# tanwanirahul/surreal

Hardware: AMD Instinct MI355X
Metric: PPO learner env-steps/sec/node (GAE+update) at 1/2/4/8 GPUs; % HBM roofline (higher is better)
Workload: dtype f32; 1 GPU; C3: synthetic PPO learner batch, reference PPO defaults (LSTM 100, horizon 5, heads 300x200, n_step 25, adapt, z-filter, 10/10 epochs), SawyerLift state dims (obs 42, act 8), 1024 segments split over 1 GPU(s) (1024 per GPU); segments_per_gpu=1024, n_step=25, env_steps_per_learn_per_gpu=25600, global_segments=1024, parallelism=single, epochs_run_last=10, ppo_mode=adapt, launch=hipGraph replay

## Files before the change

surreal_amd/csrc/lstm_mfma.hip:

```cpp
#include "smi_device.hpp"
#include "smi_internal.hpp"
#include "lstm_cell.hpp"

namespace smi {

constexpr int LR = 16;
#ifdef SMI_PROF
__device__ unsigned long long g_lstm_ticks[8];
#endif

__host__ __device__ inline int lstm_ld(int k) {
  int l = round4(k);
  if ((l & 7) != 4) l += 4;
  return l;
}

__host__ __device__ inline int lstm_q(int K) { return (((K + 3) >> 2) + 3) & ~3; }

constexpr int MAXUT = 4;
__global__ void __launch_bounds__(kWG)
lstm_fwd_kernel(LstmFwdArgs a) {
  if (a.skip && a.skip[0] != 0) return;
  const int keepS = a.keep > 0 ? a.keep : a.S;
  extern __shared__ __attribute__((aligned(16))) float sm[];
  const int H = a.H, B = a.B, G4 = 4 * H;
  const int LDH = lstm_ld(4 * lstm_q(H));
  float* hA[2] = {sm, sm + LR * LDH};
  const int lane = threadIdx.x & 63, wave = threadIdx.x >> 6;
  const int li = lane & 15, lk = lane >> 4;
  const int r0 = blockIdx.x * LR;
  const int NUT = (H + 15) >> 4;
  const int64_t BH = (int64_t)B * H;
  for (int e = threadIdx.x; e < LR * LDH; e += kWG) {
    const int r = e / LDH, k = e - r * LDH;
    const bool ok = k < H && r0 + r < B;
    const float v = ok ? a.h0[(int64_t)(r0 + r) * H + k] : 0.f;
    hA[0][e] = v;
    hA[1][e] = 0.f;
    if (ok) a.hbuf[(int64_t)(r0 + r) * H + k] = v;
  }
  float creg[MAXUT][4];
#pragma unroll
  for (int u = 0; u < MAXUT; ++u) {
    const int unit = (wave + 4 * u) * 16 + li;
#pragma unroll
    for (int i = 0; i < 4; ++i) {
      const int gr = r0 + lk * 4 + i;
      const bool ok = unit < H && gr < B;
      creg[u][i] = ok ? a.c0[(int64_t)gr * H + unit] : 0.f;
      if (ok && a.cbuf) a.cbuf[(int64_t)gr * H + unit] = creg[u][i];
    }
  }
  const float* wrow[MAXUT][4];
  float bh[MAXUT][4];
#pragma unroll
  for (int u = 0; u < MAXUT; ++u) {
    int unit = (wave + 4 * u) * 16 + li;
    unit = unit < H ? unit : H - 1;
#pragma unroll
    for (int g = 0; g < 4; ++g) {
      wrow[u][g] = a.w_hh + (int64_t)(g * H + unit) * H;
      bh[u][g] = a.b_hh[g * H + unit];
    }
  }
  const int nks = (H + 3) >> 2;
  __syncthreads();
  for (int t = 0; t < a.S; ++t) {
    const float* hp = hA[t & 1];
    float* hn = hA[(t + 1) & 1];
    float xp[MAXUT][4][4];
#pragma unroll
    for (int u = 0; u < MAXUT; ++u) {
      int unit = (wave + 4 * u) * 16 + li;
      unit = unit < H ? unit : H - 1;
#pragma unroll
      for (int i = 0; i < 4; ++i) {
        int gr = r0 + lk * 4 + i;
        gr = gr < B ? gr : B - 1;
        const float* xr = a.xproj + ((int64_t)t * B + gr) * G4 + unit;
#pragma unroll
        for (int g = 0; g < 4; ++g) xp[u][g][i] = xr[g * H];
      }
    }
    f32x4 acc[MAXUT][4];
#pragma unroll
    for (int u = 0; u < MAXUT; ++u)
#pragma unroll
      for (int g = 0; g < 4; ++g) acc[u][g] = f32x4{0.f, 0.f, 0.f, 0.f};
    const float* ap = hp + li * LDH + lk;
    int ks = 0;
    for (; ks + 4 <= nks; ks += 4) {
      float av[4], bv[MAXUT][4][4];
#pragma unroll
      for (int s = 0; s < 4; ++s) {
        const int k = (ks + s) * 4 + lk;
        const int kc = k < H ? k : H - 1;
        av[s] = ap[(ks + s) * 4];
#pragma unroll
        for (int u = 0; u < MAXUT; ++u)
#pragma unroll
          for (int g = 0; g < 4; ++g) bv[u][g][s] = wrow[u][g][kc];
      }
#pragma unroll
      for (int s = 0; s < 4; ++s)
#pragma unroll
        for (int u = 0; u < MAXUT; ++u)
#pragma unroll
          for (int g = 0; g < 4; ++g) acc[u][g] = mfma4(av[s], bv[u][g][s], acc[u][g]);
    }
    for (; ks < nks; ++ks) {
      const int k = ks * 4 + lk;
      const int kc = k < H ? k : H - 1;
      const float av = ap[ks * 4];
#pragma unroll
      for (int u = 0; u < MAXUT; ++u)
#pragma unroll
        for (int g = 0; g < 4; ++g) acc[u][g] = mfma4(av, wrow[u][g][kc], acc[u][g]);
    }
#pragma unroll
    for (int u = 0; u < MAXUT; ++u) {
      const int ut = wave + 4 * u;
      const int unit = ut * 16 + li;
      if (ut >= NUT) continue;
#pragma unroll
      for (int i = 0; i < 4; ++i) {
        const int row = lk * 4 + i, gr = r0 + row;
        const float gi = xp[u][0][i] + (acc[u][0][i] + bh[u][0]);
        const float gf = xp[u][1][i] + (acc[u][1][i] + bh[u][1]);
        const float gg = xp[u][2][i] + (acc[u][2][i] + bh[u][2]);
        const float go = xp[u][3][i] + (acc[u][3][i] + bh[u][3]);
        const float ig = sigm(gi), fg = sigm(gf), cg = ftanh(gg), og = sigm(go);
        const float c = fg * creg[u][i] + ig * cg;
        const float h = og * ftanh(c);
        const bool ok = unit < H && gr < B;
        creg[u][i] = ok ? c : 0.f;
        if (unit < H) hn[row * LDH + unit] = ok ? h : 0.f;
        if (ok) {
          a.hbuf[(int64_t)(t + 1) * BH + (int64_t)gr * H + unit] = h;
          if (a.cbuf && t < keepS) a.cbuf[(int64_t)(t + 1) * BH + (int64_t)gr * H + unit] = c;
          if (a.gates && t < keepS) {
            float* gp = a.gates + ((int64_t)t * B + gr) * G4 + unit;
            gp[0] = ig; gp[H] = fg; gp[2 * H] = cg; gp[3 * H] = og;
          }
        }
      }
    }
    __syncthreads();
  }
}



__global__ void __launch_bounds__(kWG)
lstm_bwd_kernel(LstmBwdArgs a) {
  if (a.skip && a.skip[0] != 0) return;
  extern __shared__ __attribute__((aligned(16))) float sm[];
  const int H = a.H, B = a.B, G4 = 4 * H;
  const int LDG = lstm_ld(G4);
  float* dG[2] = {sm, sm + LR * LDG};
  const int lane = threadIdx.x & 63, wave = threadIdx.x >> 6;
  const int li = lane & 15, lk = lane >> 4;
  const int r0 = blockIdx.x * LR;
  const int NUT = (H + 15) >> 4;
  const int64_t BH = (int64_t)B * H;
  for (int e = threadIdx.x; e < 2 * LR * LDG; e += kWG) sm[e] = 0.f;
  float dcreg[MAXUT][4];
  f32x4 dhrec[MAXUT];
#pragma unroll
  for (int u = 0; u < MAXUT; ++u) {
    dhrec[u] = f32x4{0.f, 0.f, 0.f, 0.f};
#pragma unroll
    for (int i = 0; i < 4; ++i) dcreg[u][i] = 0.f;
  }
  int ucl[MAXUT];
#pragma unroll
  for (int u = 0; u < MAXUT; ++u) {
    const int unit = (wave + 4 * u) * 16 + li;
    ucl[u] = unit < H ? unit : H - 1;
  }
  const int nks = G4 >> 2;
  __syncthreads();
  for (int t = a.S - 1; t >= 0; --t) {
    float* dg = dG[t & 1];
#pragma unroll
    for (int u = 0; u < MAXUT; ++u) {
      const int ut = wave + 4 * u;
      const int unit = ut * 16 + li;
      if (ut >= NUT) continue;
#pragma unroll
      for (int i = 0; i < 4; ++i) {
        const int row = lk * 4 + i;
        int gr = r0 + row;
        const bool ok = unit < H && gr < B;
        gr = gr < B ? gr : B - 1;
        const int uc = ucl[u];
        const float* gp = a.gates + ((int64_t)t * B + gr) * G4 + uc;
        const float ig = gp[0], fg = gp[H], cg = gp[2 * H], og = gp[3 * H];
        const float c = a.cbuf[(int64_t)(t + 1) * BH + (int64_t)gr * H + uc];
        const float cp = a.cbuf[(int64_t)t * BH + (int64_t)gr * H + uc];
        const float dh = a.dh[(int64_t)t * BH + (int64_t)gr * H + uc] + dhrec[u][i];
        const float tc = ftanh(c);
        const float dc = dh * og * (1.f - tc * tc) + dcreg[u][i];
        const float d_o = (dh * tc) * (og * (1.f - og));
        const float d_i = (dc * cg) * (ig * (1.f - ig));
        const float d_g = (dc * ig) * (1.f - cg * cg);
        const float d_f = (dc * cp) * (fg * (1.f - fg));
        dcreg[u][i] = ok ? dc * fg : 0.f;
        if (ok) {
          float* o = a.dgates + ((int64_t)t * B + gr) * G4 + unit;
          o[0] = d_i; o[H] = d_f; o[2 * H] = d_g; o[3 * H] = d_o;
          float* l = dg + row * LDG + unit;
          l[0] = d_i; l[H] = d_f; l[2 * H] = d_g; l[3 * H] = d_o;
        }
      }
    }
    __syncthreads();
    if (t == 0) break;
#pragma unroll
    for (int u = 0; u < MAXUT; ++u) dhrec[u] = f32x4{0.f, 0.f, 0.f, 0.f};
    const float* ap = dg + li * LDG + lk;
    int ks = 0;
    for (; ks + 8 <= nks; ks += 8) {
      float av[8], bv[MAXUT][8];
#pragma unroll
      for (int s = 0; s < 8; ++s) {
        const int k = (ks + s) * 4 + lk;
        av[s] = ap[(ks + s) * 4];
#pragma unroll
        for (int u = 0; u < MAXUT; ++u) bv[u][s] = a.w_hh[(int64_t)k * H + ucl[u]];
      }
#pragma unroll
      for (int s = 0; s < 8; ++s)
#pragma unroll
        for (int u = 0; u < MAXUT; ++u) dhrec[u] = mfma4(av[s], bv[u][s], dhrec[u]);
    }
    for (; ks < nks; ++ks) {
      const int k = ks * 4 + lk;
      const float av = ap[ks * 4];
#pragma unroll
      for (int u = 0; u < MAXUT; ++u) dhrec[u] = mfma4(av, a.w_hh[(int64_t)k * H + ucl[u]], dhrec[u]);
    }
  }
}

constexpr int kWG8 = 512;
template <int N>
__device__ __forceinline__ void load_row(const float* r, int n, float* dst) {
  static_assert(N % 4 == 0, "rows in float4 runs");
  const uintptr_t ad = reinterpret_cast<uintptr_t>(r);
  if ((ad & 15) == 0 && (n & 3) == 0) {
#pragma unroll
    for (int k = 0; k < N; k += 4) {
      const float4 v = k < n ? *reinterpret_cast<const float4*>(r + k) : float4{0.f, 0.f, 0.f, 0.f};
      dst[k] = v.x; dst[k + 1] = v.y; dst[k + 2] = v.z; dst[k + 3] = v.w;
    }
  } else if ((ad & 7) == 0 && (n & 1) == 0) {
#pragma unroll
    for (int k = 0; k < N; k += 2) {
      const float2 v = k < n ? *reinterpret_cast<const float2*>(r + k) : float2{0.f, 0.f};
      dst[k] = v.x; dst[k + 1] = v.y;
    }
  } else {
#pragma unroll
    for (int k = 0; k < N; ++k) dst[k] = k < n ? r[k] : 0.f;
  }
}

constexpr int LR4 = 4;
constexpr int LSTM_HQ = 4;

__device__ __forceinline__ f32x4 mfma4x64(float a, float b, f32x4 c) {
  return __builtin_amdgcn_mfma_f32_4x4x1f32(a, b, c, 4, 0, 0);
}

__device__ __attribute__((aligned(16))) float g_lstm_zero4[4] = {0.f, 0.f, 0.f, 0.f};
template <int N, int V>
__device__ __forceinline__ void load_row_v(const float* r, int n, float* dst) {
  static_assert(N % 4 == 0 && (V == 4 || V == 2), "vector rows");
#pragma unroll
  for (int k = 0; k < N; k += V) {
    const float* src = k < n ? r + k : g_lstm_zero4;
    if constexpr (V == 4) {
      const float4 v = *reinterpret_cast<const float4*>(src);
      dst[k] = v.x; dst[k + 1] = v.y; dst[k + 2] = v.z; dst[k + 3] = v.w;
    } else {
      const float2 v = *reinterpret_cast<const float2*>(src);
      dst[k] = v.x; dst[k + 1] = v.y;
    }
  }
}

template <int N>
__device__ __forceinline__ void load_col(const float* t, int n, int ld, uint32_t zoff, int col,
                                         float* dst) {
#pragma unroll
  for (int k = 0; k < N; ++k) {
    const uint32_t row = k < n ? (uint32_t)(k * ld) : zoff;
    dst[k] = t[row + (uint32_t)col];
  }
}

template <int KP, int KX, bool VF = false, bool IMG = false>
__global__ void __launch_bounds__(kWG8)
lstm_fwd_r4_kernel(LstmFwdArgs a) {
  if (a.skip && a.skip[0] != 0) return;
  LSTM_T0();
  const int keepS = a.keep > 0 ? a.keep : a.S;
  constexpr int KXS = KX > 0 ? KX : 8;
  __shared__ __attribute__((aligned(16))) float hS[2][LR4 * KP];
  __shared__ __attribute__((aligned(16))) float xS[2][LR4 * KXS];
  __shared__ float pre[LR4][4 * KP];
  const int H = a.H, B = a.B, G4 = 4 * H;
  const int tid = threadIdx.x, lane = tid & 63, wave = tid >> 6;
  const int r0 = blockIdx.x * LR4;
  const int64_t BH = (int64_t)B * H;
  const int col = wave * 64 + lane;
  const bool cact = wave * 64 < G4;
  const int colc = col < G4 ? col : G4 - 1;
  float w[KP];
  float wx[KXS];
  float bh = a.b_hh[colc];
  if constexpr (KX > 0) bh += a.b_ih[colc];
  if constexpr (IMG) {
    load_col<KP>(a.w_hh, H, G4, (uint32_t)(H * G4), colc, w);
    if constexpr (KX > 0) load_col<KX>(a.w_ih, a.din, G4, (uint32_t)((a.din + H) * G4), colc, wx);
  } else if constexpr (VF) {
    load_row_v<KP, 4>(a.w_hh + (int64_t)colc * H, H, w);
    if constexpr (KX > 0) load_row_v<KX, 2>(a.w_ih + (int64_t)colc * a.din, a.din, wx);
  } else {
    load_row<KP>(a.w_hh + (int64_t)colc * H, H, w);
    if constexpr (KX > 0) load_row<KX>(a.w_ih + (int64_t)colc * a.din, a.din, wx);
  }
  const int xr = tid / KXS, xk = tid - (tid / KXS) * KXS;
  const bool xown = KX > 0 && tid < LR4 * KXS;
  const int64_t xoff0 = (int64_t)min(r0 + xr, B - 1) * a.ldx + min(xk, a.din - 1);
  const bool xval = xk < a.din;
  auto xload = [&](int t) -> float { return a.x[(int64_t)t * B * a.ldx + xoff0]; };
  float xnext = 0.f, x0 = 0.f;
  if constexpr (KX > 0) {
    x0 = xload(0);
    xnext = xload(a.S > 1 ? 1 : 0);
  }
  const bool cell = tid < LR4 * H;
  const int crow = cell ? tid / H : 0;
  const int cunit = cell ? tid - crow * H : 0;
  const int cgr = r0 + crow;
  const bool cok = cell && cgr < B;
  const float c0v = a.c0[(int64_t)min(cgr, B - 1) * H + cunit];
  static_assert(LR4 * KP <= kWG8, "one h0 slot per thread");
  const int he = min(tid, LR4 * KP - 1);
  const int hr = he / KP, hk = he - hr * KP;
  float h0v = a.h0[(int64_t)min(r0 + hr, B - 1) * H + min(hk, H - 1)];
  asm volatile("" : "+v"(h0v));
  if constexpr (KX > 0) asm volatile("" : "+v"(x0));
  if constexpr (KX > 0) {
    if (xown && a.S > 0) xS[0][xr * KXS + xk] = xval ? x0 : 0.f;
  }
  float creg = cok ? c0v : 0.f;
  if (cok && a.cbuf) a.cbuf[(int64_t)cgr * H + cunit] = creg;
  if (tid < LR4 * KP) {
    const bool ok = hk < H && r0 + hr < B;
    const float v = ok ? h0v : 0.f;
    hS[0][he] = v;
    hS[1][he] = 0.f;
    if (ok) a.hbuf[(int64_t)(r0 + hr) * H + hk] = v;
  }
  int64_t xoff[4];
#pragma unroll
  for (int i = 0; i < 4; ++i) {
    const int gr = r0 + i < B ? r0 + i : B - 1;
    xoff[i] = (int64_t)gr * G4 + colc;
  }
  float xp[4] = {0.f, 0.f, 0.f, 0.f};
  if (KX == 0 && a.S > 0) {
#pragma unroll
    for (int i = 0; i < 4; ++i) xp[i] = a.xproj[xoff[i]];
  }
  __syncthreads();
  LSTM_TICK(6);
  f32x4 acc[8];
#pragma unroll
  for (int j = 0; j < 8; ++j) acc[j] = f32x4{0.f, 0.f, 0.f, 0.f};
  auto x_part = [&](int tt) {
    if constexpr (KX > 0) {
      const float4* xr4 = reinterpret_cast<const float4*>(xS[tt & 1] + (lane & 3) * KXS);
      constexpr int NQX = KX / 4;
      float4 q[LSTM_HQ];
#pragma unroll
      for (int j = 0; j < LSTM_HQ && j < NQX; ++j) q[j] = xr4[j];
#pragma unroll
      for (int j = 0; j < NQX; ++j) {
        const float4 u = q[j % LSTM_HQ];
        const int ab = (j & 1) * 4;
        acc[ab + 0] = mfma4x64(u.x, wx[4 * j + 0], acc[ab + 0]);
        acc[ab + 1] = mfma4x64(u.y, wx[4 * j + 1], acc[ab + 1]);
        acc[ab + 2] = mfma4x64(u.z, wx[4 * j + 2], acc[ab + 2]);
        acc[ab + 3] = mfma4x64(u.w, wx[4 * j + 3], acc[ab + 3]);
        if (j + LSTM_HQ < NQX) q[j % LSTM_HQ] = xr4[j + LSTM_HQ];
      }
      __builtin_amdgcn_sched_group_barrier(0x100, LSTM_HQ < NQX ? LSTM_HQ : NQX, 0);
#pragma unroll
      for (int j = 0; j < NQX; ++j) {
        __builtin_amdgcn_sched_group_barrier(0x008, 4, 0);
        if (j + LSTM_HQ < NQX) __builtin_amdgcn_sched_group_barrier(0x100, 1, 0);
      }
    }
  };
  if (cact && a.S > 0) x_part(0);
  for (int t = 0; t < a.S; ++t) {
    const float* hp = hS[t & 1];
    float* hn = hS[(t + 1) & 1];
    if (cact) {
      const float4* hr = reinterpret_cast<const float4*>(hp + (lane & 3) * KP);
      constexpr int NQ = KP / 4;
      float4 q[LSTM_HQ];
#pragma unroll
      for (int j = 0; j < LSTM_HQ; ++j) q[j] = hr[j];
#pragma unroll
      for (int j = 0; j < NQ; ++j) {
        const float4 u = q[j % LSTM_HQ];
        const int ab = (j & 1) * 4;
        acc[ab + 0] = mfma4x64(u.x, w[4 * j + 0], acc[ab + 0]);
        acc[ab + 1] = mfma4x64(u.y, w[4 * j + 1], acc[ab + 1]);
        acc[ab + 2] = mfma4x64(u.z, w[4 * j + 2], acc[ab + 2]);
        acc[ab + 3] = mfma4x64(u.w, w[4 * j + 3], acc[ab + 3]);
        if (j + LSTM_HQ < NQ) q[j % LSTM_HQ] = hr[j + LSTM_HQ];
      }
      __builtin_amdgcn_sched_group_barrier(0x100, LSTM_HQ, 0);
#pragma unroll
      for (int j = 0; j < NQ; ++j) {
        __builtin_amdgcn_sched_group_barrier(0x008, 4, 0);
        if (j + LSTM_HQ < NQ) __builtin_amdgcn_sched_group_barrier(0x100, 1, 0);
      }
      const f32x4 sum = ((acc[0] + acc[1]) + (acc[2] + acc[3])) +
                        ((acc[4] + acc[5]) + (acc[6] + acc[7]));
      if (col < G4) {
#pragma unroll
        for (int i = 0; i < 4; ++i) pre[i][col] = xp[i] + (sum[i] + bh);
      }
      if (KX == 0 && t + 1 < a.S) {
#pragma unroll
        for (int i = 0; i < 4; ++i) xp[i] = a.xproj[(int64_t)(t + 1) * B * G4 + xoff[i]];
      }
    }
    if constexpr (KX > 0) {
      if (xown && t + 1 < a.S) xS[(t + 1) & 1][xr * KXS + xk] = xval ? xnext : 0.f;
      if (xown && t + 2 < a.S) xnext = xload(t + 2);
    }
    LSTM_TICK(0);
    __syncthreads();
    if (cact) {
#pragma unroll
      for (int j = 0; j < 8; ++j) acc[j] = f32x4{0.f, 0.f, 0.f, 0.f};
      if (t + 1 < a.S) x_part(t + 1);
    }
    if (cell) {
      const float ig = sigm(pre[crow][cunit]), fg = sigm(pre[crow][H + cunit]);
      const float cg = ftanh(pre[crow][2 * H + cunit]), og = sigm(pre[crow][3 * H + cunit]);
      const float c = fg * creg + ig * cg;
      const float h = og * ftanh(c);
      creg = cok ? c : 0.f;
      hn[crow * KP + cunit] = cok ? h : 0.f;
      if (cok) {
        a.hbuf[(int64_t)(t + 1) * BH + (int64_t)cgr * H + cunit] = h;
        if (a.cbuf && t < keepS) a.cbuf[(int64_t)(t + 1) * BH + (int64_t)cgr * H + cunit] = c;
        if (a.gates && t < keepS) {
          float* gp = a.gates + ((int64_t)t * B + cgr) * G4 + cunit;
          gp[0] = ig; gp[H] = fg; gp[2 * H] = cg; gp[3 * H] = og;
        }
      }
    }
    LSTM_TICK(1);
    __syncthreads();
    LSTM_TICK(2);
  }
}

struct BpttIn { float ig, fg, cg, og, c, cp, dh; };
struct BpttFac { float tc, omt, fo, fi, fgg, ff; };

__device__ __forceinline__ BpttFac bptt_factors(const BpttIn& s) {
#pragma clang fp contract(off)
  BpttFac f;
  f.tc = ftanh(s.c);
  f.omt = fmaf(-f.tc, f.tc, 1.f);
  f.fo = s.og * (1.f - s.og);
  f.fi = s.ig * (1.f - s.ig);
  f.fgg = fmaf(-s.cg, s.cg, 1.f);
  f.ff = s.fg * (1.f - s.fg);
  return f;
}

__device__ __forceinline__ float bptt_cell(const BpttIn& s, const BpttFac& f, float dhr, float dcreg,
                                           float d[4]) {
#pragma clang fp contract(off)
  const float dh = s.dh + dhr;
  const float dc = fmaf(dh * s.og, f.omt, dcreg);
  d[3] = (dh * f.tc) * f.fo;
  d[0] = (dc * s.cg) * f.fi;
  d[2] = (dc * s.ig) * f.fgg;
  d[1] = (dc * s.cp) * f.ff;
  return dc * s.fg;
}

__device__ float g_lstm_zero_row[128];
template <int KW>
__global__ void __launch_bounds__(kWG8, KW <= 32 ? 4 : 2)
lstm_bwd_r4_kernel(LstmBwdArgs a) {
  if (a.skip && a.skip[0] != 0) return;
  LSTM_T0();
  constexpr int G4P = 4 * 128 + KW;
  constexpr int WPG = KW <= 32 ? 8 : 4;
  __shared__ __attribute__((aligned(16))) float dG[LR4 * G4P];
  __shared__ float red[8][LR4][64];
  const int H = a.H, B = a.B, G4 = 4 * H;
  const int tid = threadIdx.x, lane = tid & 63;
  const int wave = __builtin_amdgcn_readfirstlane(tid >> 6);
  const int r0 = blockIdx.x * LR4;
  const int64_t BH = (int64_t)B * H, BG4 = (int64_t)B * G4;
  const int kw = (G4 + WPG - 1) / WPG;
  const int ug = wave / WPG, kp = wave - ug * WPG;
  const int k0 = kp * kw;
  const int unit = ug * 64 + lane;
  const int uc = unit < H ? unit : H - 1;
  for (int e = tid; e < LR4 * G4P; e += kWG8) dG[e] = 0.f;
  for (int e = tid; e < 8 * LR4 * 64; e += kWG8) (&red[0][0][0])[e] = 0.f;
  const bool cell = tid < LR4 * H;
  const int crow = cell ? tid / H : 0;
  const int cunit = cell ? tid - crow * H : 0;
  const int cgr = r0 + crow;
  const bool cok = cell && cgr < B;
  const int64_t grc = cgr < B ? cgr : B - 1;
  const int cug = cunit >> 6, cl = cunit & 63;
  const int64_t goff = grc * G4 + cunit, hoff = grc * H + cunit;
  auto fetch = [&](int t, BpttIn& s) {
    const float* gp = a.gates + ((int64_t)t * BG4 + goff);
    s.ig = gp[0]; s.fg = gp[H]; s.cg = gp[2 * H]; s.og = gp[3 * H];
    const int64_t o = (int64_t)t * BH + hoff;
    s.c = a.cbuf[o + BH];
    s.cp = a.cbuf[o];
    s.dh = a.dh[o];
  };
  BpttIn sa, sb;
  fetch(a.S - 1, sa);
  fetch(a.S > 1 ? a.S - 2 : 0, sb);
  float w[KW];
  const int jn = min(kw, G4 - k0);
#pragma unroll
  for (int j = 0; j < KW; ++j) {
    const bool in = j < jn;
    const float* base = in ? a.w_hh : g_lstm_zero_row;
    const uint32_t ro = in ? (uint32_t)((k0 + j) * H) : 0u;
    w[j] = base[ro + (uint32_t)uc];
  }
  asm volatile("" : "+v"(sa.ig), "+v"(sa.fg), "+v"(sa.cg), "+v"(sa.og), "+v"(sa.c), "+v"(sa.cp),
               "+v"(sa.dh));
  asm volatile("" : "+v"(sb.ig), "+v"(sb.fg), "+v"(sb.cg), "+v"(sb.og), "+v"(sb.c), "+v"(sb.cp),
               "+v"(sb.dh));
  BpttFac f = bptt_factors(sa);
  float dcreg = 0.f;
  __builtin_amdgcn_s_waitcnt(0x0F70);
  __syncthreads();
  LSTM_TICK(7);
  auto cells = [&](const BpttIn& x, float d[4]) __attribute__((always_inline)) {
    if (cell) {
      float r[WPG];
#pragma unroll
      for (int p = 0; p < WPG; ++p) r[p] = red[cug * WPG + p][crow][cl];
      float dhr = 0.f;
#pragma unroll
      for (int p = 0; p < WPG; ++p) dhr += r[p];
      const float dcf = bptt_cell(x, f, dhr, dcreg, d);
      dcreg = cok ? dcf : 0.f;
      float* l = dG + crow * G4P + cunit;
      l[0] = cok ? d[0] : 0.f; l[H] = cok ? d[1] : 0.f;
      l[2 * H] = cok ? d[2] : 0.f; l[3 * H] = cok ? d[3] : 0.f;
    }
    LSTM_TICK(3);
    __syncthreads();
    LSTM_TICK(4);
  };
  auto store = [&](int t, const float d[4]) __attribute__((always_inline)) {
    if (cok) {
      float* o = a.dgates + ((int64_t)t * BG4 + (int64_t)cgr * G4 + cunit);
      o[0] = d[0]; o[H] = d[1]; o[2 * H] = d[2]; o[3 * H] = d[3];
    }
  };
  auto step = [&](int t, BpttIn& x, BpttIn& y) __attribute__((always_inline)) {
    float d[4] = {0.f, 0.f, 0.f, 0.f};
    cells(x, d);
    f32x4 acc[8];
#pragma unroll
    for (int j = 0; j < 8; ++j) acc[j] = f32x4{0.f, 0.f, 0.f, 0.f};
    constexpr int NQ = KW / 4, LQ = 4;
    const float4* dr = reinterpret_cast<const float4*>(dG + (lane & 3) * G4P + k0);
    float4 q[LQ];
#pragma unroll
    for (int j = 0; j < LQ && j < NQ; ++j) q[j] = dr[j];
#pragma unroll
    for (int j = 0; j < NQ; ++j) {
      const float4 u = q[j % LQ];
      if (j + LQ < NQ) q[j % LQ] = dr[j + LQ];
      const int a0 = (j & 1) * 4;
      acc[a0 + 0] = mfma4x64(u.x, w[4 * j + 0], acc[a0 + 0]);
      acc[a0 + 1] = mfma4x64(u.y, w[4 * j + 1], acc[a0 + 1]);
      acc[a0 + 2] = mfma4x64(u.z, w[4 * j + 2], acc[a0 + 2]);
      acc[a0 + 3] = mfma4x64(u.w, w[4 * j + 3], acc[a0 + 3]);
      if (j == 1) {
        store(t, d);
        fetch(t > 1 ? t - 2 : 0, x);
      }
      __builtin_amdgcn_sched_barrier(0);
    }
    asm volatile("" : "+v"(y.ig), "+v"(y.fg), "+v"(y.cg), "+v"(y.og), "+v"(y.c), "+v"(y.cp),
                 "+v"(y.dh));
    f = bptt_factors(y);
    asm volatile("" : "+v"(f.tc), "+v"(f.omt), "+v"(f.fo), "+v"(f.fi), "+v"(f.fgg), "+v"(f.ff));
    const f32x4 sum = ((acc[0] + acc[1]) + (acc[2] + acc[3])) +
                      ((acc[4] + acc[5]) + (acc[6] + acc[7]));
#pragma unroll
    for (int i = 0; i < 4; ++i) red[wave][i][lane] = sum[i];
    LSTM_TICK(5);
    __syncthreads();
  };
  int t = a.S - 1;
  for (int i = t >> 1; i > 0; --i, t -= 2) {
    step(t, sa, sb);
    step(t - 1, sb, sa);
  }
  float d[4] = {0.f, 0.f, 0.f, 0.f};
  if (t == 1) {
    step(1, sa, sb);
    cells(sb, d);
  } else {
    cells(sa, d);
  }
  store(0, d);
}

static int device_cus() {
  static int cus = 0;
  if (!cus) {
    int dev = 0;
    (void)hipGetDevice(&dev);
    if (hipDeviceGetAttribute(&cus, hipDeviceAttributeMultiprocessorCount, dev) != hipSuccess || cus < 1)
      cus = 256;
  }
  return cus;
}
static bool lstm_valu(int B, int H) { return H >= 1 && H <= 128 && B <= device_cus(); }
bool lstm_fwd_image_ok(int B, int H) { return H >= 1 && H <= 128 && B >= 1 && !lstm_valu(B, H); }

__global__ void __launch_bounds__(kWG)
lstm_weight_image_kernel(const float* __restrict__ w_ih, const float* __restrict__ w_hh, int din,
                         int H, float* __restrict__ image) {
  const int G4 = 4 * H, nih = G4 * din, nw = nih + G4 * H;
  const int o = blockIdx.x * kWG + threadIdx.x;
  if (o >= nw + G4) return;
  if (o < nih) {
    const int k = o / G4, col = o - k * G4;
    image[o] = w_ih[col * din + k];
  } else if (o < nw) {
    const int k = (o - nih) / G4, col = (o - nih) - k * G4;
    image[o] = w_hh[col * H + k];
  } else {
    image[o] = 0.f;
  }
}

int launch_lstm_weight_image(const float* w_ih, const float* w_hh, int din, int H, float* image,
                             hipStream_t st) {
  if (H < 1 || H > 128 || din < 1 || din > 4096)
    return set_error(SMI_E_ARG, "lstm_weight_image: H must be in [1, 128], din in [1, 4096]");
  const int n = 4 * H * (din + H + 1);
  hipLaunchKernelGGL(lstm_weight_image_kernel, dim3((n + kWG - 1) / kWG), dim3(kWG), 0, st, w_ih,
                     w_hh, din, H, image);
  return check_launch("lstm_weight_image_kernel");
}

#ifdef SMI_PROF
extern "C" int smi_lstm_phase_ticks(unsigned long long* out ) {
  if (hipMemcpyFromSymbol(out, HIP_SYMBOL(g_lstm_ticks), sizeof(g_lstm_ticks)) != hipSuccess)
    return SMI_E_LAUNCH;
  static const unsigned long long zero[8] = {0, 0, 0, 0, 0, 0, 0, 0};
  return hipMemcpyToSymbol(HIP_SYMBOL(g_lstm_ticks), zero, sizeof(zero)) == hipSuccess ? SMI_OK
                                                                                        : SMI_E_LAUNCH;
}
#endif

int64_t lstm_fwd_lds(int H) { return (int64_t)2 * LR * lstm_ld(4 * lstm_q(H)) * 4; }
int64_t lstm_bwd_lds(int H) { return (int64_t)2 * LR * lstm_ld(4 * H) * 4; }

static bool r4_vf(const LstmFwdArgs& a, bool fused_x) {
  auto al = [](const void* p, uintptr_t m) { return (reinterpret_cast<uintptr_t>(p) & m) == 0; };
  if (a.H % 4 != 0 || !al(a.w_hh, 15)) return false;
  return !fused_x || (a.din % 2 == 0 && a.din >= 2 && al(a.w_ih, 7));
}

int launch_lstm_fwd(const float* xproj, const float* w_hh, const float* b_hh, const float* h0,
                    const float* c0, int S, int B, int H, float* hbuf, float* cbuf, float* gates,
                    hipStream_t st, const int* skip, int keep, bool image) {
  if (B <= 0 || S < 0) return SMI_OK;
  if (H < 1 || H > 256) return set_error(SMI_E_ARG, "lstm: hidden size must be in [1, 256]");
  if (image && !lstm_fwd_image_ok(B, H)) return SMI_E_NOFIT;
  LstmFwdArgs a{xproj, w_hh, b_hh, h0, c0, S, B, H, hbuf, cbuf, gates, skip};
  a.keep = keep;
  const int kslot = ktime_begin(st);
  struct End { int s; hipStream_t st; double f;
               ~End() { ktime_end(s, KT_LSTM_FWD, f, st); } } end_{kslot, st, 8.0 * B * H * (double)H * S};
  if (lstm_valu(B, H)) return check_launch(lstm_v_fwd(a, 0, st));
  if (H <= 128) {
    const dim3 g4((B + LR4 - 1) / LR4);
    const bool vf = r4_vf(a, false);
#define SMI_R4F(KP_)                                                                        \
    do {                                                                                    \
      if (image) {                                                                          \
        hipLaunchKernelGGL((lstm_fwd_r4_kernel<KP_, 0, false, true>), g4, dim3(kWG8), 0,    \
                           st, a);                                                          \
        return check_launch("lstm_fwd_r4_kernel<" #KP_ ",0,img>");                          \
      } else if (vf) {                                                                      \
        hipLaunchKernelGGL((lstm_fwd_r4_kernel<KP_, 0, true>), g4, dim3(kWG8), 0, st, a);   \
        return check_launch("lstm_fwd_r4_kernel<" #KP_ ",0,vf>");                           \
      } else {                                                                              \
        hipLaunchKernelGGL((lstm_fwd_r4_kernel<KP_, 0>), g4, dim3(kWG8), 0, st, a);         \
        return check_launch("lstm_fwd_r4_kernel<" #KP_ ",0>");                              \
      }                                                                                     \
    } while (0)
    if (H <= 32) SMI_R4F(32);
    else if (H <= 64) SMI_R4F(64);
    else if (H <= 104) SMI_R4F(104);
    else SMI_R4F(128);
#undef SMI_R4F
  }
  const size_t lds = (size_t)lstm_fwd_lds(H);
  const dim3 grid((B + LR - 1) / LR);
  allow_lds(lstm_fwd_kernel, lds);
  hipLaunchKernelGGL(lstm_fwd_kernel, grid, dim3(kWG), lds, st, a);
  return check_launch("lstm_fwd_kernel<4>");
}

int launch_lstm_fwd_x(const float* x, int64_t ldx, int din, const float* w_ih, const float* b_ih,
                      const float* w_hh, const float* b_hh, const float* h0, const float* c0,
                      int S, int B, int H, float* hbuf, float* cbuf, float* gates,
                      hipStream_t st, const int* skip, int keep, bool image) {
  if (B <= 0 || S <= 0) return SMI_OK;
  if (!lstm_fwd_x_fuses(din, H)) return SMI_E_NOFIT;
  const bool valu = lstm_valu(B, H);
  if (image && valu) return SMI_E_NOFIT;
  if (image && w_hh != w_ih + (int64_t)4 * H * din)
    return set_error(SMI_E_ARG, "lstm: W_hhT must follow W_ihT in the weight image");
  if (valu && lstm_fwd_v_lds(S, din <= 48 ? 48 : 64, (4 * H + 63) & ~63) > kVxMax)
    return SMI_E_NOFIT;
  LstmFwdArgs a{nullptr, w_hh, b_hh, h0, c0, S, B, H, hbuf, cbuf, gates, skip,
                x, ldx, din, w_ih, b_ih, keep};
  const int kslot = ktime_begin(st);
  struct End { int s; hipStream_t st; double f;
               ~End() { ktime_end(s, KT_LSTM_FWD, f, st); } } end_{
      kslot, st, 8.0 * B * H * (double)(H + din) * S};
  if (valu) return check_launch(lstm_v_fwd(a, din <= 48 ? 48 : 64, st));
  const dim3 g4((B + LR4 - 1) / LR4);
  const bool vf = r4_vf(a, true);
#define SMI_R4X(KP_, KX_)                                                                     \
  do {                                                                                        \
    if (image) {                                                                              \
      hipLaunchKernelGGL((lstm_fwd_r4_kernel<KP_, KX_, false, true>), g4, dim3(kWG8), 0, st,  \
                         a);                                                                  \
      return check_launch("lstm_fwd_r4_kernel<" #KP_ "," #KX_ ",img>");                       \
    } else if (vf) {                                                                          \
      hipLaunchKernelGGL((lstm_fwd_r4_kernel<KP_, KX_, true>), g4, dim3(kWG8), 0, st, a);     \
      return check_launch("lstm_fwd_r4_kernel<" #KP_ "," #KX_ ",vf>");                        \
    } else {                                                                                  \
      hipLaunchKernelGGL((lstm_fwd_r4_kernel<KP_, KX_>), g4, dim3(kWG8), 0, st, a);           \
      return check_launch("lstm_fwd_r4_kernel<" #KP_ "," #KX_ ">");                           \
    }                                                                                         \
  } while (0)
  if (din <= 48) {
    if (H <= 64) SMI_R4X(64, 48);
    else SMI_R4X(104, 48);
  } else {
    if (H <= 64) SMI_R4X(64, 64);
    else SMI_R4X(104, 64);
  }
#undef SMI_R4X
}

int lstm_bwd_q_form(int B, int H, const float* w_hh) {
  if (!lstm_valu(B, H) || !lstm_bwd_q_ok(H, w_hh)) return 0;
  return H <= 64 ? 16 : H <= 100 ? 25 : 32;
}

bool lstm_fwd_x_dual_fits(int B0, int B1, int S, int H, int din) {
  if (din < 1 || din > 64 || H < 1 || H > 104 || B0 <= 0 || B1 <= 0)
    return false;
  if (!lstm_valu(B0 + B1, H)) return false;
  return lstm_fwd_v_lds(S, din <= 48 ? 48 : 64, (4 * H + 63) & ~63) <= kVxMax;
}

int launch_lstm_fwd_x_dual(const LstmFwdArgs& a0, const LstmFwdArgs& a1, hipStream_t st) {
  const int H = a0.H, din = a0.din;
  const int smax = a0.S > a1.S ? a0.S : a1.S;
  if (a0.S <= 0 && a1.S <= 0) return SMI_OK;
  if (a0.S <= 0 || a1.S <= 0) return SMI_E_NOFIT;
  if (a0.H != a1.H || a0.din != a1.din || !lstm_fwd_x_dual_fits(a0.B, a1.B, smax, H, din))
    return SMI_E_NOFIT;
  const int kx = din <= 48 ? 48 : 64;
  const int kslot = ktime_begin(st);
  const char* form = lstm_q_fwd_dual(a0, a1, kx, st);
  ktime_end(kslot, KT_LSTM_FWD,
            8.0 * H * (double)(H + din) * ((double)a0.B * a0.S + (double)a1.B * a1.S), st);
  return check_launch(form);
}

int launch_lstm_bwd(const float* dh, const float* gates, const float* cbuf, const float* w_hh,
                    int S, int B, int H, float* dgates, hipStream_t st, const int* skip) {
  if (B <= 0 || S <= 0) return SMI_OK;
  if (H < 1 || H > 256) return set_error(SMI_E_ARG, "lstm: hidden size must be in [1, 256]");
  LstmBwdArgs a{dh, gates, cbuf, w_hh, S, B, H, dgates, skip};
  const int kslot = ktime_begin(st);
  struct End { int s; hipStream_t st; double f;
               ~End() { ktime_end(s, KT_LSTM_BWD, f, st); } } end_{kslot, st,
                                                                 8.0 * B * H * (double)H * (S - 1)};
  if (lstm_valu(B, H)) return check_launch(lstm_v_bwd(a, st));
  if (H <= 128) {
    const int nu = (H + 63) / 64, wpg = 8 / nu;
    const int kw = (4 * H + wpg - 1) / wpg;
    const dim3 g4((B + LR4 - 1) / LR4);
#define SMI_R4B(KW_)                                                              \
    do {                                                                          \
      hipLaunchKernelGGL(lstm_bwd_r4_kernel<KW_>, g4, dim3(kWG8), 0, st, a);      \
      return check_launch("lstm_bwd_r4_kernel<" #KW_ ">");                        \
    } while (0)
    if (kw <= 32) SMI_R4B(32);
    else if (kw <= 104) SMI_R4B(104);
    else SMI_R4B(128);
#undef SMI_R4B
  }
  const size_t lds = (size_t)lstm_bwd_lds(H);
  if (lds > 160 * 1024) return set_error(SMI_E_NOFIT, "lstm: hidden size too large for LDS");
  const dim3 grid((B + LR - 1) / LR);
  allow_lds(lstm_bwd_kernel, lds);
  hipLaunchKernelGGL(lstm_bwd_kernel, grid, dim3(kWG), lds, st, a);
  return check_launch("lstm_bwd_kernel<4>");
}


}
```

Before: 4.223 million env-steps/s.

## Dedicate eighth wave to prefetching LSTM input and raise compute-wave priority

In the fused-input LSTM forward kernel, wave 7 (otherwise idle since 4*KP ≤ 448) becomes a producer. It loads x for upcoming timesteps into the double-buffered LDS slot and matches the consumer waves' two barriers per step, then exits. The compute waves no longer issue x global loads or LDS stores in their recurrent loop, and waves 4 to 6 get raised scheduling priority. The change also adds profiling-only wall-clock tick counters. The risk is barrier-count mismatch: wave 7 returns after the loop while the others continue, which relies on hardware barrier semantics for exited waves.

```diff
diff --git a/surreal_amd/csrc/lstm_mfma.hip b/surreal_amd/csrc/lstm_mfma.hip
--- a/surreal_amd/csrc/lstm_mfma.hip
+++ b/surreal_amd/csrc/lstm_mfma.hip
@@ -7,6 +7,18 @@
 constexpr int LR = 16;
 #ifdef SMI_PROF
 __device__ unsigned long long g_lstm_ticks[8];
+__device__ unsigned long long g_lstm_ticks_w4[8];
+#define LSTM_TICK_F(id)                                                     \
+  do {                                                                      \
+    LSTM_TICK(id);                                                          \
+    if (blockIdx.x == 0 && threadIdx.x == 256) {                            \
+      const unsigned long long n_ = wall_clock64();                         \
+      g_lstm_ticks_w4[id] += n_ - t_prev_;                                  \
+      t_prev_ = n_;                                                         \
+    }                                                                       \
+  } while (0)
+#else
+#define LSTM_TICK_F(id) (void)0
 #endif
 
 __host__ __device__ inline int lstm_ld(int k) {
@@ -311,9 +323,45 @@
   __shared__ __attribute__((aligned(16))) float xS[2][LR4 * KXS];
   __shared__ float pre[LR4][4 * KP];
   const int H = a.H, B = a.B, G4 = 4 * H;
-  const int tid = threadIdx.x, lane = tid & 63, wave = tid >> 6;
+  const int tid = threadIdx.x, lane = tid & 63;
+  const int wave = KX > 0 ? __builtin_amdgcn_readfirstlane(tid >> 6) : tid >> 6;
   const int r0 = blockIdx.x * LR4;
   const int64_t BH = (int64_t)B * H;
+  if constexpr (KX > 0) {
+    static_assert(4 * KP <= 448 && (LR4 * KXS) % 64 == 0, "the eighth wave is free");
+    if (wave == 7) {
+      constexpr int NX = LR4 * KXS / 64;
+      int64_t xo[NX];
+      bool xv[NX];
+#pragma unroll
+      for (int i = 0; i < NX; ++i) {
+        const int e = lane + 64 * i, r = e / KXS, k = e - r * KXS;
+        xo[i] = (int64_t)min(r0 + r, B - 1) * a.ldx + min(k, a.din - 1);
+        xv[i] = k < a.din;
+      }
+      const int64_t sx = (int64_t)B * a.ldx;
+      const int64_t t1 = (int64_t)min(1, a.S - 1) * sx;
+      float xc[NX], xn[NX];
+#pragma unroll
+      for (int i = 0; i < NX; ++i) xc[i] = a.x[xo[i]];
+#pragma unroll
+      for (int i = 0; i < NX; ++i) xn[i] = a.x[t1 + xo[i]];
+#pragma unroll
+      for (int i = 0; i < NX; ++i) xS[0][lane + 64 * i] = xv[i] ? xc[i] : 0.f;
+      __syncthreads();
+      for (int t = 0; t < a.S; ++t) {
+#pragma unroll
+        for (int i = 0; i < NX; ++i) xS[(t + 1) & 1][lane + 64 * i] = xv[i] ? xn[i] : 0.f;
+        const int64_t tn = (int64_t)min(t + 2, a.S - 1) * sx;
+#pragma unroll
+        for (int i = 0; i < NX; ++i) xn[i] = a.x[tn + xo[i]];
+        __syncthreads();
+        __syncthreads();
+      }
+      return;
+    }
+    if (wave >= 4) __builtin_amdgcn_s_setprio(1);
+  }
   const int col = wave * 64 + lane;
   const bool cact = wave * 64 < G4;
   const int colc = col < G4 ? col : G4 - 1;
@@ -331,16 +379,6 @@
     load_row<KP>(a.w_hh + (int64_t)colc * H, H, w);
     if constexpr (KX > 0) load_row<KX>(a.w_ih + (int64_t)colc * a.din, a.din, wx);
   }
-  const int xr = tid / KXS, xk = tid - (tid / KXS) * KXS;
-  const bool xown = KX > 0 && tid < LR4 * KXS;
-  const int64_t xoff0 = (int64_t)min(r0 + xr, B - 1) * a.ldx + min(xk, a.din - 1);
-  const bool xval = xk < a.din;
-  auto xload = [&](int t) -> float { return a.x[(int64_t)t * B * a.ldx + xoff0]; };
-  float xnext = 0.f, x0 = 0.f;
-  if constexpr (KX > 0) {
-    x0 = xload(0);
-    xnext = xload(a.S > 1 ? 1 : 0);
-  }
   const bool cell = tid < LR4 * H;
   const int crow = cell ? tid / H : 0;
   const int cunit = cell ? tid - crow * H : 0;
@@ -352,10 +390,6 @@
   const int hr = he / KP, hk = he - hr * KP;
   float h0v = a.h0[(int64_t)min(r0 + hr, B - 1) * H + min(hk, H - 1)];
   asm volatile("" : "+v"(h0v));
-  if constexpr (KX > 0) asm volatile("" : "+v"(x0));
-  if constexpr (KX > 0) {
-    if (xown && a.S > 0) xS[0][xr * KXS + xk] = xval ? x0 : 0.f;
-  }
   float creg = cok ? c0v : 0.f;
   if (cok && a.cbuf) a.cbuf[(int64_t)cgr * H + cunit] = creg;
   if (tid < LR4 * KP) {
@@ -377,7 +411,7 @@
     for (int i = 0; i < 4; ++i) xp[i] = a.xproj[xoff[i]];
   }
   __syncthreads();
-  LSTM_TICK(6);
+  LSTM_TICK_F(6);
   f32x4 acc[8];
 #pragma unroll
   for (int j = 0; j < 8; ++j) acc[j] = f32x4{0.f, 0.f, 0.f, 0.f};
@@ -443,11 +477,7 @@
         for (int i = 0; i < 4; ++i) xp[i] = a.xproj[(int64_t)(t + 1) * B * G4 + xoff[i]];
       }
     }
-    if constexpr (KX > 0) {
-      if (xown && t + 1 < a.S) xS[(t + 1) & 1][xr * KXS + xk] = xval ? xnext : 0.f;
-      if (xown && t + 2 < a.S) xnext = xload(t + 2);
-    }
-    LSTM_TICK(0);
+    LSTM_TICK_F(0);
     __syncthreads();
     if (cact) {
 #pragma unroll
@@ -470,9 +500,9 @@
         }
       }
     }
-    LSTM_TICK(1);
+    LSTM_TICK_F(1);
     __syncthreads();
-    LSTM_TICK(2);
+    LSTM_TICK_F(2);
   }
 }
 
@@ -679,6 +709,13 @@
 }
 
 #ifdef SMI_PROF
+extern "C" int smi_lstm_phase_ticks_w4(unsigned long long* out ) {
+  if (hipMemcpyFromSymbol(out, HIP_SYMBOL(g_lstm_ticks_w4), sizeof(g_lstm_ticks_w4)) != hipSuccess)
+    return SMI_E_LAUNCH;
+  static const unsigned long long zero[8] = {0, 0, 0, 0, 0, 0, 0, 0};
+  return hipMemcpyToSymbol(HIP_SYMBOL(g_lstm_ticks_w4), zero, sizeof(zero)) == hipSuccess
+             ? SMI_OK : SMI_E_LAUNCH;
+}
 extern "C" int smi_lstm_phase_ticks(unsigned long long* out ) {
   if (hipMemcpyFromSymbol(out, HIP_SYMBOL(g_lstm_ticks), sizeof(g_lstm_ticks)) != hipSuccess)
     return SMI_E_LAUNCH;
```

After: 4.242 million env-steps/s (median of 6 runs). About the same (+0.4%).
